# Liupeter01/Software-Rasterizer

Hardware: AMD Instinct MI355X
Metric: frames_per_sec (higher is better)
Workload: dtype f32

## Files before the change

software-rasterizer_amd/csrc/srz_api.hip:

```cpp
#include <dlfcn.h>

#include <algorithm>
#include <cmath>
#include <cstdio>
#include <cstdlib>
#include <cstring>
#include <new>
#include <string>
#include <vector>

#include "srz_device.h"

using namespace srz;

namespace {
std::string g_create_error;

struct EventPair {
  hipEvent_t t0, t1, t2, t3;
  bool detailed;
};

struct BatchDesc {
  int32_t shader, tex_id;
// ... 450 lines not shown
  }
  return SRZ_OK;
}

void end_clear_plan(srz_frameset *fs, const ClearPlan &p, hipStream_t s) {
  if (p.count) ++fs->clear_tune.renders;
  if (p.stamp) launch_clear_tune(fs->clear_tune.d_ctl, fs->clear_tune.h_wgs, s);
  if (p.rebase) launch_clear_rebase(fs->clear_tune.d_ctl, s);
}

struct RenderPlan {
  Pass pass;
  hipStream_t s;
  bool side, turns, vertex_setup;
  ClearPlan clear;
  EventPair *ep;
};

int enqueue_sub_batch(srz_ctx *ctx, srz_frameset *fs, const RenderPlan &r, RenderArgs &a, int f0, int n, int part) {
  const bool stats = r.pass.kind == Pass::COUNTING;
  const hipStream_t s = r.s;
  const size_t tpf = (size_t)fs->n_local_bands * fs->tiles_x;
  RenderArgs v = a;
  if (n != fs->n_frames) {
    const int fa = r.pass.f_begin + f0;
    v.frames += fa, v.n_frames = (uint32_t)n;
    v.vis += (size_t)fa * tpf * ((size_t)TILE * TILE);
    v.tile_info += (size_t)fa * tpf;
    v.out += (size_t)fa * a.frame_stride;
    v.work_cap = (uint32_t)((size_t)(n < 8 ? n : (n + 7) / 8) * tpf);
  }
  const uint32_t tiles = (uint32_t)((size_t)n * tpf);
  if (r.vertex_setup) launch_chunks(v, n, fs->max_tris, s);
  else launch_setup(v, n, fs->max_tris, stats, s);
  launch_bin(v, n, fs->max_tris, s);
  if (!fs->pool_sized && !stats) {
    HIP_TRY(ctx, copy_demand(fs, part, s));
    HIP_TRY(ctx, hipStreamSynchronize(s));
    const uint32_t need = max_pool_demand(fs, part, part + 1);
    if (need > fs->pool_sub_cap) {
      if (int rc = grow_pool(ctx, fs, need, 8u)) return rc;
      a.pool = v.pool = fs->d_pool, a.pool_sub_cap = v.pool_sub_cap = fs->pool_sub_cap;
      HIP_TRY(ctx, hipMemsetAsync(fs->d_pool_heads, 0, sizeof(uint32_t) * CNT_STRIDE * fs->pool_n_sub, s));
      launch_bin(v, n, fs->max_tris, s);
    }
  }
  if (r.pass.kind == Pass::SIZE_ONLY) return SRZ_OK;
  if (r.ep) HIP_TRY(ctx, hipEventRecord(r.ep->t1, s));
  const unsigned ev = r.side ? ctx->ev_next++ % srz_ctx::EV_RING : 0u;
  if (r.side) {
    HIP_TRY(ctx, hipEventRecord(ctx->ev_fork[ev], s));
    HIP_TRY(ctx, hipStreamWaitEvent(ctx->stream2, ctx->ev_fork[ev], 0));
    launch_clear(v, tiles, ctx->stream2, r.clear.wgs);
    HIP_TRY(ctx, copy_demand(fs, part, ctx->stream2));
    HIP_TRY(ctx, hipEventRecord(ctx->ev_join[ev], ctx->stream2));
  }
  launch_raster(v, n, stats, s);
  if (r.turns) {
    HIP_TRY(ctx, hipEventRecord(ctx->ev_raster[ctx->raster_next++ % srz_ctx::EV_RING], s));
    ctx->raster_last_stream = s, ctx->raster_valid = true;
  }
  if (r.ep) HIP_TRY(ctx, hipEventRecord(r.ep->t2, s));
  if (r.pass.kind == Pass::VISIBILITY) launch_visibility(v, tiles, s);
  else launch_shade(v, tiles, stats, fs->fast_kinds, fs->any_generic, fs->approx_shade, s);
  if (r.side) HIP_TRY(ctx, hipStreamWaitEvent(s, ctx->ev_join[ev], 0));
  else if (!raster_four_waves(v))
    HIP_TRY(ctx, copy_demand(fs, part, s));
  return SRZ_OK;
}

int check_renderable(srz_ctx *ctx, const srz_frameset *fs) {
  if (fs->shard_rank != ctx->shard_rank || fs->shard_world != ctx->shard_world)
    return fail(ctx, SRZ_E_INVALID, "frameset was created under a different shard (call srz_set_shard before srz_frameset_create)");
  if (fs->update_failed) return fail(ctx, SRZ_E_NOMEM, "the last update of this set failed (out of memory): update it again or destroy it");
  return SRZ_OK;
}

int render_impl(srz_ctx *ctx, srz_frameset *fs, float *d_out, uint32_t flags_or, hipStream_t s, Pass pass) {
  const bool stats = pass.kind == Pass::COUNTING, size_only = pass.kind == Pass::SIZE_ONLY;
  if (int rc = check_renderable(ctx, fs)) return rc;
  if (pass.kind == Pass::COLOUR || stats)
    if (int rc = resolve_shading(ctx, fs, s)) return rc;
  const uint32_t need = max_pool_demand(fs, 0, srz_frameset::DEMAND_PARTS);
  if (need > fs->pool_sub_cap)
    if (int rc = grow_pool(ctx, fs, need, 4u)) return rc;
  RenderArgs a = make_args(ctx, fs, d_out, flags_or, pass);
  if (!size_only) fs->last_flags = flags_or, fs->rendered = true;
  EventPair ep{};
  const bool timed = ctx->timing != 0 && !stats && !size_only && ctx->ev_used.size() < 65536, detailed = timed && ctx->timing >= 2;
  if (timed)
    if (int rc = begin_timing(ctx, ep, detailed, s)) return rc;
  if (stats) HIP_TRY(ctx, hipMemsetAsync(ctx->d_stats, 0, ST_COUNT * sizeof(unsigned long long), s));
  if (fs->max_tris == 0) {
    HIP_TRY(ctx, hipMemsetAsync(fs->d_work_count, 0, sizeof(uint32_t) * CNT_STRIDE * N_WORK_LISTS, s));
    HIP_TRY(ctx, hipMemsetAsync(fs->d_pool_heads, 0, sizeof(uint32_t) * CNT_STRIDE * fs->pool_n_sub, s));
    HIP_TRY(ctx, hipMemsetAsync(fs->d_slow_count, 0, 2 * sizeof(uint32_t), s));
  }
  const bool turns = !stats && !size_only && fs->max_tiles >= 8192;
  if (turns && !ctx->ev_raster[0])
    if (int rc = create_side(ctx, "render: raster events", nullptr, false, ctx->ev_raster)) return rc;
  if (turns && ctx->raster_valid && ctx->raster_last_stream != s) {
    HIP_TRY(ctx, hipStreamWaitEvent(s, ctx->ev_raster[(ctx->raster_next + srz_ctx::EV_RING - 1) % srz_ctx::EV_RING], 0));
    a.other_streams = 1u;
  }
  const bool vertex_setup = fs->d_draws != nullptr && !stats;
  if (fs->d_draws) launch_vertex(fs->d_draws, fs->n_draws, fs->max_faces, fs->d_tris, fs->d_tri_pos, fs->d_frames, vertex_setup ? fs->d_bbox : nullptr, s);
  const bool any_fused = any_frame_has(fs, flags_or, SRZ_FUSED_CLEAR), side = any_fused && fs->max_tiles >= 8192 && !size_only;
  if (side && !ctx->stream2)
    if (int rc = create_side(ctx, "render: clear stream", &ctx->stream2, true, ctx->ev_fork, ctx->ev_join)) return rc;
  if (!side && any_fused) a.clear_in_raster = 1u;
  RenderPlan r{pass, s, side, turns, vertex_setup, ClearPlan{}, detailed ? &ep : nullptr};
  if (side)
    if (int rc = plan_clear(ctx, fs, pass, detailed, s, r.clear)) return rc;
  a.clear_wgs_dev = r.clear.dev_wgs;
  const int n_all = pass.f_count < 0 ? fs->n_frames : pass.f_count;
  const int chunk = sub_batch_frames(ctx, fs, n_all, stats || detailed);
  for (int f0 = 0, part = 0; f0 < n_all; f0 += chunk, ++part)
    if (int rc = enqueue_sub_batch(ctx, fs, r, a, f0, std::min(chunk, n_all - f0), part)) return rc;
  if (!stats) fs->pool_sized = true;
  end_clear_plan(fs, r.clear, s);
  if (timed) {
    HIP_TRY(ctx, hipEventRecord(ep.t3, s));
    ctx->ev_used.push_back(ep);
  }
  HIP_TRY(ctx, hipGetLastError());
  return SRZ_OK;
}

int render_entry(const char *name, srz_ctx *ctx, srz_frameset *fs, void *d_out, size_t out_bytes, uint32_t flags, void *stream, Pass pass) {
  if (!ctx) return SRZ_E_INVALID;
  const std::string fn(name);
  if (!fs || !d_out) return fail(ctx, SRZ_E_INVALID, fn + ": null frameset / output");
  if (out_bytes < srz_frameset_out_bytes(ctx, fs)) return fail(ctx, SRZ_E_INVALID, fn + ": output buffer too small");
  if (((uintptr_t)d_out & 15u) != 0) return fail(ctx, SRZ_E_INVALID, fn + ": output must be 16-byte aligned");
  HIP_TRY(ctx, hipSetDevice(ctx->device));
  return render_impl(ctx, fs, (float *)d_out, flags & FRAME_FLAGS, pick_stream(ctx, stream), pass);
}

int read_stats(srz_ctx *ctx, hipStream_t s, srz_stats *st) {
  unsigned long long h[ST_COUNT];
  HIP_TRY(ctx, hipMemcpyAsync(h, ctx->d_stats, sizeof h, hipMemcpyDeviceToHost, s));
  HIP_TRY(ctx, hipStreamSynchronize(s));
  st->n_tris = h[ST_TRIS], st->n_culled = h[ST_CULLED], st->pixel_tests = h[ST_PIXEL_TESTS];
  st->fragments = h[ST_FRAGMENTS], st->shaded = h[ST_SHADED], st->visible = h[ST_VISIBLE];
  st->visible_textured = h[ST_VISIBLE_TEX];
  std::memcpy(ctx->dbg, h, sizeof h);
  return SRZ_OK;
// ... 241 lines not shown
      o += sb.n_tris;
    }
    if (fr.n_lights) std::memcpy(&fs->h_lights[d.light_off], fr.lights, sizeof(srz_light) * fr.n_lights);
  }
  classify_frames(fs);
  if (draws) {
    fs->h_draws = *draws, fs->n_draws = (uint32_t)draws->size();
    for (const DrawDesc &dd : *draws) fs->max_faces = std::max(fs->max_faces, dd.n_faces);
  }
  auto up16 = [](size_t v) { return (v + 15) & ~(size_t)15; };
  fs->dyn_lights_off = up16(sizeof(FrameDesc) * (size_t)n_frames);
  fs->dyn_draws_off = up16(fs->dyn_lights_off + sizeof(srz_light) * (size_t)light_off);
  fs->dyn_bytes = fs->dyn_draws_off + sizeof(DrawDesc) * fs->h_draws.size();
  auto dev_alloc = [&](void **p, size_t bytes) { return hipMalloc(p, std::max<size_t>(bytes, 256)); };
  hipError_t e = hipSuccess;
#define FS_TRY(expr)                                                                                                   \
  if (e == hipSuccess) e = (expr)
  FS_TRY(dev_alloc((void **)&fs->d_dyn, fs->dyn_bytes));
  if (e == hipSuccess) {
    fs->d_frames = reinterpret_cast<FrameDesc *>(fs->d_dyn);
    fs->d_lights = reinterpret_cast<srz_light *>(fs->d_dyn + fs->dyn_lights_off);
    if (draws) fs->d_draws = reinterpret_cast<DrawDesc *>(fs->d_dyn + fs->dyn_draws_off);
  }
  FS_TRY(dev_alloc((void **)&fs->d_tris, sizeof(srz_tri) * tri_off));
  if (!fs->tris_aos) FS_TRY(dev_alloc((void **)&fs->d_tri_pos, sizeof(float) * TRI_POS_F * tri_off + 16));
  FS_TRY(dev_alloc((void **)&fs->d_bbox, sizeof(BBox) * tri_off));
  FS_TRY(dev_alloc((void **)&fs->d_chunk_rows, sizeof(uint32_t) * (tri_off / 64 + (size_t)n_frames + 1)));
  FS_TRY(dev_alloc((void **)&fs->d_band_desc, sizeof(uint32_t) * group_off * fs->n_local_bands));
  FS_TRY(dev_alloc((void **)&fs->d_band_ent, sizeof(uint2) * group_off * ENT_PER_GROUP));
  FS_TRY(dev_alloc((void **)&fs->d_tri_batch, sizeof(uint16_t) * tri_off));
  fs->max_tiles = (uint32_t)n_frames * fs->n_local_bands * fs->tiles_x;
  {
    const uint64_t n_wgs = (uint64_t)((n_frames + 7) / 8 * 8) * fs->n_local_bands;
    uint32_t n_sub = 1;
    while (n_sub < 64u && (uint64_t)n_sub * 256u <= n_wgs) n_sub *= 2u;
    fs->pool_n_sub = n_sub;
    const uint64_t cap = std::min<uint64_t>((4ull * tri_off + 4096u) / n_sub + 64u, 0xfffffff0ull / n_sub);
    fs->pool_sub_cap = (uint32_t)cap;
    FS_TRY(dev_alloc((void **)&fs->d_pool, sizeof(uint32_t) * cap * n_sub));
    FS_TRY(dev_alloc((void **)&fs->d_pool_heads, sizeof(uint32_t) * CNT_STRIDE * 64));
    FS_TRY(hipHostMalloc((void **)&fs->h_pool_heads, sizeof(uint32_t) * CNT_STRIDE * 64 * srz_frameset::DEMAND_PARTS, hipHostMallocMapped | hipHostMallocCoherent));
    if (e == hipSuccess) std::memset(fs->h_pool_heads, 0, sizeof(uint32_t) * CNT_STRIDE * 64 * srz_frameset::DEMAND_PARTS);
    FS_TRY(dev_alloc((void **)&fs->clear_tune.d_ctl, sizeof(ClearCtl)));
    if (e == hipSuccess) FS_TRY(hipMemset(fs->clear_tune.d_ctl, 0, sizeof(ClearCtl)));
    FS_TRY(hipHostMalloc((void **)&fs->clear_tune.h_wgs, 64, hipHostMallocMapped | hipHostMallocCoherent));
    if (e == hipSuccess) *fs->clear_tune.h_wgs = 0u;
    FS_TRY(dev_alloc((void **)&fs->d_tile_info, sizeof(uint2) * fs->max_tiles));
    FS_TRY(dev_alloc((void **)&fs->d_slow_list, sizeof(uint32_t) * fs->max_tiles));
    FS_TRY(dev_alloc((void **)&fs->d_slow_count, 2 * sizeof(uint32_t)));
    FS_TRY(dev_alloc((void **)&fs->d_redo_list, sizeof(uint4) * fs->max_tiles));
  }
  FS_TRY(dev_alloc((void **)&fs->d_vis, sizeof(uint32_t) * (size_t)fs->max_tiles * ((size_t)TILE * TILE)));
  FS_TRY(ensure_worklists(fs));
  FS_TRY(dev_alloc((void **)&fs->d_work_count, sizeof(uint32_t) * CNT_STRIDE * N_WORK_LISTS));
  FS_TRY(dev_alloc((void **)&fs->d_sdesc, sizeof(ShadeDescG) * fs->h_batches.size()));
  std::vector<uint8_t> h_dyn(fs->dyn_bytes);
  stage_dyn(fs, h_dyn.data());
  FS_TRY(hipMemcpy(fs->d_dyn, h_dyn.data(), fs->dyn_bytes, hipMemcpyHostToDevice));
  if (tri_off) {
    if (copy_tris) FS_TRY(hipMemcpy(fs->d_tris, h_tris.data(), sizeof(srz_tri) * tri_off, hipMemcpyHostToDevice));
    if (!h_pos.empty()) FS_TRY(hipMemcpy(fs->d_tri_pos, h_pos.data(), sizeof(float) * h_pos.size(), hipMemcpyHostToDevice));
    FS_TRY(hipMemcpy(fs->d_tri_batch, h_tb.data(), sizeof(uint16_t) * tri_off, hipMemcpyHostToDevice));
  }
#undef FS_TRY
  if (e != hipSuccess) {
    free_frameset_buffers(fs);
    delete fs;
    return fail(ctx, e == hipErrorOutOfMemory ? SRZ_E_NOMEM : SRZ_E_NODEVICE,
                std::string("srz_frameset_create: ") + hipGetErrorString(e));
  }
  *out = fs;
  return SRZ_OK;
}

static int size_pool_at_create(srz_ctx *ctx, srz_frameset **out) {
  srz_frameset *fs = *out;
  if (fs->pool_sized) return SRZ_OK;
  int rc = render_impl(ctx, fs, nullptr, 0, ctx->stream, Pass::size_only());
  if (rc == SRZ_OK && hipStreamSynchronize(ctx->stream) != hipSuccess) rc = fail(ctx, SRZ_E_NODEVICE, "srz_frameset_create: the binning pass failed");
  if (rc != SRZ_OK) {
    srz_frameset_destroy(ctx, fs);
    *out = nullptr;
  }
  return rc;
}

int srz_frameset_create(srz_ctx *ctx, const srz_frame *frames, int n_frames, srz_frameset **out) {
  int rc = build_frameset(ctx, frames, n_frames, out, true);
  return rc == SRZ_OK ? size_pool_at_create(ctx, out) : rc;
}

int srz_mesh_upload(srz_ctx *ctx, int mesh_id, const srz_vertex *verts, uint32_t n_verts, const uint32_t *faces, uint32_t n_faces) {
  if (!ctx) return SRZ_E_INVALID;
  if (mesh_id < 0 || mesh_id >= MAX_MESH || !verts || !faces || n_verts == 0) return fail(ctx, SRZ_E_INVALID, "srz_mesh_upload: bad arguments");
  for (uint32_t i = 0; i < 3u * n_faces; ++i)
    if (faces[i] >= n_verts) return fail(ctx, SRZ_E_INVALID, "srz_mesh_upload: face index out of range");
  HIP_TRY(ctx, hipSetDevice(ctx->device));
  srz_ctx::MeshSlot m;
  HIP_TRY(ctx, hipMalloc(&m.d_verts, sizeof(srz_vertex) * n_verts));
  hipError_t e = hipMalloc(&m.d_faces, sizeof(uint32_t) * 3 * (n_faces ? n_faces : 1));
  if (e == hipSuccess) e = hipMemcpy(m.d_verts, verts, sizeof(srz_vertex) * n_verts, hipMemcpyHostToDevice);
  if (e == hipSuccess && n_faces) e = hipMemcpy(m.d_faces, faces, sizeof(uint32_t) * 3 * n_faces, hipMemcpyHostToDevice);
  if (e != hipSuccess) {
    (void)hipFree(m.d_verts), (void)hipFree(m.d_faces);
    return fail(ctx, SRZ_E_NOMEM, std::string("srz_mesh_upload: ") + hipGetErrorString(e));
  }
  m.n_verts = n_verts, m.n_faces = n_faces;
// ... 914 lines not shown
```

software-rasterizer_amd/csrc/srz_device.h:

```cpp
#pragma once
#include <hip/hip_runtime.h>
#include <stdint.h>

#include "../../include/srz.h"

namespace srz {

constexpr int TILE = 32;
constexpr int BAND = 32;
constexpr int KEY_STRIDE = TILE + 1;
constexpr int LDS_STRIDE = 32;
#ifndef SRZ_BAND_ROT
#define SRZ_BAND_ROT 5
#endif
__host__ __device__ inline int band_rot(int world) { return (SRZ_BAND_ROT % world) ? SRZ_BAND_ROT : (SRZ_BAND_ROT ? 1 : 0); }
__host__ __device__ inline int band_of(int lb, int rank, int world) {
  if (world == 1) return lb;
  int j = (rank - band_rot(world) * lb) % world;
  return lb * world + (j < 0 ? j + world : j);
}
__host__ __device__ inline int rank_of_band(int b, int world) { return (b + band_rot(world) * (b / world)) % world; }
constexpr uint32_t NO_TRI = 0xffffffffu;
constexpr uint32_t CNT_STRIDE = 32;
constexpr uint32_t FD_FAST_SHADE = 0x100u, FD_NL_SHIFT = 9;
// ... 56 lines not shown
  uint32_t n_local_bands;
  uint32_t chunk_off;
  uint32_t group_off;
};

enum { ST_TRIS = 0, ST_CULLED, ST_PIXEL_TESTS, ST_FRAGMENTS, ST_SHADED, ST_VISIBLE, ST_VISIBLE_TEX,
       ST_DBG_CYC_A, ST_DBG_CYC_B, ST_DBG_CYC_C, ST_DBG_MAX_WAVE, ST_DBG_IEEE_TILES, ST_DBG_BLOCKS, ST_COUNT };

struct RenderArgs {
  const FrameDesc *frames;
  const srz_tri *tris;
  const float *tri_pos;
  uint32_t pos_stride;
  const BBox *bbox;
  uint32_t *chunk_rows;
  uint32_t *band_desc;
  uint2 *band_ent;
  const uint16_t *tri_batch;
  const srz_light *lights;
  const ShadeDescG *sdesc;
  uint32_t *pool;
  uint32_t *pool_heads;
  uint32_t *pool_demand;
  uint32_t pool_sub_cap, pool_sub_mask;
  uint2 *tile_info;
  uint32_t *slow_list;
  uint32_t *slow_count;
  uint32_t other_streams;
  uint32_t clear_in_raster;
  uint32_t force_ordered;
  uint32_t any_ordered;
  uint32_t force_generic;
  uint32_t any_generic;
  uint4 *redo_list;
  uint32_t *redo_count;
  uint32_t *vis;
  uint4 *worklist;
  uint64_t kind_slots;
  uint32_t *work_count;
  uint32_t work_cap;
  uint32_t tiles_x, n_local_bands, n_frames;
  float *out;
  uint64_t frame_stride;
  uint32_t local_rows;
  int32_t shard_rank, shard_world;
  uint32_t flags_or;
  unsigned long long *stats;
  const uint32_t *clear_wgs_dev;
};

constexpr int CLEAR_CANDS = 3, CLEAR_TUNE_BLOCK = 3, CLEAR_TUNE_RENDERS = 2 * CLEAR_CANDS * CLEAR_TUNE_BLOCK;
constexpr uint32_t CLEAR_CAND[CLEAR_CANDS] = {96, 128, 256};
constexpr uint32_t CLEAR_GRID_MAX = 256, CLEAR_GRID_DEFAULT = 96;
struct ClearCtl {
  uint32_t wgs;
  uint32_t cur, pos, phase, done, alive;
  uint32_t n[CLEAR_CANDS];
  unsigned long long last;
  float t[CLEAR_CANDS][4];
  float score[CLEAR_CANDS];
};
void launch_clear_tune(ClearCtl *ctl, uint32_t *h_wgs, hipStream_t s);
void launch_clear_rebase(ClearCtl *ctl, hipStream_t s);

void launch_vertex(const DrawDesc *draws, uint32_t n_draws, uint32_t max_faces, srz_tri *tris, float *tri_pos, const FrameDesc *frames,
                   BBox *bbox_out, hipStream_t s);
void launch_chunks(const RenderArgs &a, int n_frames, uint32_t max_tris, hipStream_t s);
void launch_setup(const RenderArgs &a, int n_frames, uint32_t max_tris, bool stats, hipStream_t s);
void launch_bin(const RenderArgs &a, int n_frames, uint32_t max_tris, hipStream_t s);
void launch_raster(const RenderArgs &a, int n_frames, bool stats, hipStream_t s);
bool raster_four_waves(const RenderArgs &a);
void launch_clear(const RenderArgs &a, uint32_t max_tiles, hipStream_t s, uint32_t wgs);
void launch_shade(const RenderArgs &a, uint32_t max_tiles, bool stats, uint32_t kinds, bool any_generic, bool approx, hipStream_t s);
void launch_visibility(const RenderArgs &a, uint32_t max_tiles, hipStream_t s);
struct ShadeVisArgs {
  const FrameDesc *frames;
  const srz_tri *tris;
  const uint16_t *tri_batch;
  const srz_light *lights;
  const ShadeDescG *sdesc;
  const float *vis;
  float *out;
  uint64_t frame_stride;
  uint32_t local_rows, tiles_x, n_local_bands, n_frames;
  int32_t shard_rank, shard_world;
  uint32_t flags_or, in_place;
  uint32_t any_generic;
  uint32_t *redo_list;
  uint32_t *redo_count;
};
void launch_shade_vis(const ShadeVisArgs &a, uint32_t kinds, bool any_generic, bool approx, hipStream_t s);
void launch_resolve8(const float *planes, uint8_t *out, uint32_t n_frames, uint32_t rows, uint32_t W, uint64_t frame_stride,
                     hipStream_t s);
void launch_deinterleave(const void *gathered, void *full, uint32_t world, uint32_t n_fp, uint32_t bands_per_rank, uint32_t row_bytes,
                         hipStream_t s);
constexpr uint32_t SPARSE_HEADER = 16;
constexpr uint32_t SPARSE_NONE = 0xffffffffu;
constexpr uint32_t SPARSE_UNPACK_WGS = 2048;
struct SparseArgs {
  const void *shard;
  uint8_t *msg;
  const uint2 *tile_info;
  const FrameDesc *frames;
  uint32_t *row_cnt;
  uint32_t flags_or;
  uint32_t n_frames, n_local_bands, bands_per_rank, tiles_x;
// ... 14 lines not shown
```

software-rasterizer_amd/csrc/srz_kernels.hip:

```cpp
#include "srz_device.h"

#include <algorithm>
#include <cstdio>
#include <cstdlib>
#include <type_traits>

#pragma clang fp contract(off)

namespace srz {

#define SRZ_CAS __attribute__((address_space(4)))
template <typename T> __device__ __forceinline__ const SRZ_CAS T *as_const(const T *p) { return (const SRZ_CAS T *)(p); }
typedef float f32x4 __attribute__((ext_vector_type(4)));
typedef unsigned int u32x2 __attribute__((ext_vector_type(2)));
typedef unsigned int u32x4 __attribute__((ext_vector_type(4)));

__device__ __forceinline__ float sse_max(float a, float b) { return a > b ? a : b; }
__device__ __forceinline__ float sse_min(float a, float b) { return a < b ? a : b; }
__device__ __forceinline__ float std_max(float a, float b) { return (a < b) ? b : a; }
__device__ __forceinline__ float std_clamp(float v, float lo, float hi) { return (v < lo) ? lo : (hi < v) ? hi : v; }
__device__ __forceinline__ float fmsubf(float a, float b, float c) { return __builtin_fmaf(a, b, -c); }
__device__ __forceinline__ float fmaf_(float a, float b, float c) { return __builtin_fmaf(a, b, c); }

__device__ __forceinline__ uint32_t f2u_(float f) { return __builtin_bit_cast(uint32_t, f); }
// ... 432 lines not shown
      run += (uint32_t)__builtin_amdgcn_readlane((int)incl, 63);
    }
    if (lane == 0 && run > ENT_PER_GROUP) s_misc[0] = 1u;
  }
  __syncthreads();
  const bool raw = s_misc[0] != 0u;
  uint32_t tpk[GROUP_K];
#pragma unroll
  for (int k = 0; k < (int)GROUP_K; ++k) {
    const uint32_t t = t0 + (uint32_t)k * 256u + (uint32_t)tid;
    tpk[k] = t;
    if (packed && keep[k]) tpk[k] = t | ((uint32_t)as_const(a.tri_batch)[tri_off + t] << PACK_IDX_BITS);
  }
  uint32_t *desc = a.band_desc + (size_t)group * nlb;
  for (uint32_t i = (uint32_t)tid; i < nlb; i += 256u) desc[i] = raw ? DESC_RAW : ((s_off[i] << 16) | s_cnt[i]);
  if (!raw) {
    uint2 *ent = a.band_ent + (size_t)group * ENT_PER_GROUP;
#pragma unroll
    for (int k = 0; k < (int)GROUP_K; ++k) {
      const uint32_t xr = (uint32_t)((int)bb[k].sx >> 5) | ((uint32_t)((int)bb[k].ex >> 5) << 16);
      float m = 0.0f;
      const bool tight = P != nullptr && nb[k] > 0 &&
                         tight_margin(P[k][0], P[k][1], P[k][3], P[k][4], P[k][6], P[k][7],
                                      (P[k][3] - P[k][0]) * (P[k][7] - P[k][1]) - (P[k][4] - P[k][1]) * (P[k][6] - P[k][0]), bb[k].sx,
                                      bb[k].sy, bb[k].ex, bb[k].ey, m);
      for (int j = 0; j < nb[k]; ++j) {
        uint32_t xr_j = xr;
        if (tight) {
          const int b = band_of(lb0[k] + j, rank, world);
          int X0 = bb[k].sx, X1 = bb[k].ex;
          float mn, mx;
          slab_extent(P[k][0], P[k][1], P[k][3], P[k][4], P[k][6], P[k][7], (float)max(b * BAND, (int)bb[k].sy) - m,
                      (float)min(b * BAND + BAND - 1, (int)bb[k].ey) + m, mn, mx);
          clip_range(X0, X1, mn, mx, m);
          xr_j = X0 <= X1 ? ((uint32_t)(X0 >> 5) | ((uint32_t)(X1 >> 5) << 16)) : 1u;
        }
        ent[atomicAdd(&s_fill[lb0[k] + j], 1u)] = make_uint2(tpk[k], xr_j);
      }
    }
  }
  __syncthreads();
}

__device__ __forceinline__ void chunk_rows_store(const RenderArgs &a, const uint32_t chunk_off, const uint32_t t, const uint32_t n_tris,
                                                 const bool keep, const BBox &bb) {
  int lo = keep ? (int)bb.sy : 0x7fff, hi = keep ? (int)bb.ey : -1;
  for (int o = 32; o > 0; o >>= 1) lo = min(lo, __shfl_xor(lo, o)), hi = max(hi, __shfl_xor(hi, o));
  if ((threadIdx.x & 63) == 0 && (t & ~63u) < n_tris) a.chunk_rows[chunk_off + t / 64u] = ((uint32_t)lo & 0xffffu) | ((uint32_t)hi << 16);
}

__device__ __forceinline__ void reset_render_counters(const RenderArgs &a) {
  if (threadIdx.x < N_WORK_LISTS) a.work_count[threadIdx.x * CNT_STRIDE] = 0u, a.work_count[threadIdx.x * CNT_STRIDE + 1] = 0u;
  if (threadIdx.x <= a.pool_sub_mask) a.pool_heads[threadIdx.x * CNT_STRIDE] = 0u;
  if (threadIdx.x == 0) *a.slow_count = 0u, *a.redo_count = 0u;
}

template <bool STATS>
__global__ __launch_bounds__(256) void k_setup(RenderArgs a, BBox *bbox_out) {
  __shared__ uint32_t s_cnt[MAX_LOCAL_BANDS], s_off[MAX_LOCAL_BANDS], s_fill[MAX_LOCAL_BANDS], s_misc[2];
  if (blockIdx.x == 0 && blockIdx.y == 0) reset_render_counters(a);
  const SRZ_CAS FrameDesc *fd = as_const(a.frames) + blockIdx.y;
  const int W = fd->width, H = fd->height;
  const uint32_t n_tris = fd->n_tris, tri_off = fd->tri_off;
  const float ex = fd->eye[0], ey = fd->eye[1], ez = fd->eye[2];
  unsigned long long n_culled = 0, tests = 0;
  const uint32_t n_groups = (n_tris + GROUP_TRIS - 1u) / GROUP_TRIS;
  for (uint32_t g = blockIdx.x; g < n_groups; g += gridDim.x) {
    const uint32_t t0 = g * GROUP_TRIS;
    float P[GROUP_K][9];
#pragma unroll
    for (int k = 0; k < (int)GROUP_K; ++k) {
      const uint32_t t = t0 + (uint32_t)k * 256u + threadIdx.x;
      load_pos9(as_const(a.tri_pos) + (size_t)(tri_off + (t < n_tris ? t : 0u)) * a.pos_stride, P[k]);
    }
    BBox bb[GROUP_K];
    bool keep[GROUP_K];
#pragma unroll
    for (int k = 0; k < (int)GROUP_K; ++k) {
      const uint32_t t = t0 + (uint32_t)k * 256u + threadIdx.x;
      const bool live = t < n_tris;
      keep[k] = setup_triangle(P[k], W, H, ex, ey, ez, live, bb[k]);
      if (STATS) {
        if (keep[k])
          tests += (unsigned long long)(bb[k].ex - bb[k].sx + 1) * (unsigned long long)(bb[k].ey - bb[k].sy + 1);
        else if (live)
          n_culled++;
      }
      if (live) bbox_out[tri_off + t] = bb[k];
      chunk_rows_store(a, fd->chunk_off, t, n_tris, keep[k], bb[k]);
    }
    bucket_group(a, fd->n_local_bands, fd->group_off + g, t0, (fd->flags & FD_PACKED) != 0u, tri_off, bb, keep, P, s_cnt, s_off, s_fill, s_misc);
  }
  if (STATS) {
    if (n_culled) atomicAdd(&a.stats[ST_CULLED], n_culled);
    if (tests) atomicAdd(&a.stats[ST_PIXEL_TESTS], tests);
    if (blockIdx.x == 0 && threadIdx.x == 0) atomicAdd(&a.stats[ST_TRIS], (unsigned long long)n_tris);
  }
}

__global__ __launch_bounds__(256) void k_chunks(RenderArgs a) {
  __shared__ uint32_t s_cnt[MAX_LOCAL_BANDS], s_off[MAX_LOCAL_BANDS], s_fill[MAX_LOCAL_BANDS], s_misc[2];
  if (blockIdx.x == 0 && blockIdx.y == 0) reset_render_counters(a);
  const SRZ_CAS FrameDesc *fd = as_const(a.frames) + blockIdx.y;
  const uint32_t n_tris = fd->n_tris, tri_off = fd->tri_off;
  const SRZ_CAS u32x2 *bbox = as_const(reinterpret_cast<const u32x2 *>(a.bbox + tri_off));
  const uint32_t n_groups = (n_tris + GROUP_TRIS - 1u) / GROUP_TRIS;
  for (uint32_t g = blockIdx.x; g < n_groups; g += gridDim.x) {
// ... 1187 lines not shown
              const bool pass = inside & !(z > zold);
              if (pass) {
                zl[li] = z;
                il[li] = idx | S_CLASS_BIT;
              }
              if (STATS) n_frag += inside ? 1 : 0, n_shaded += pass ? 1 : 0;
            }
          }
        }
      }
    }
    __builtin_amdgcn_wave_barrier();
    bool any_owner = false;
    for (int it = 0; it < 4; ++it) {
      const uint4 q = *reinterpret_cast<const uint4 *>(&il[(it * 8 + (lane >> 3)) * LDS_STRIDE + (lane & 7) * 4]);
      any_owner |= (q.x & q.y & q.z & q.w) != NO_TRI;
    }
    const bool tile_has_owner = __ballot(any_owner) != 0ull;
    const bool vec_ok = (W & 3) == 0;
    if (tile_has_owner || fused) {
      const float4 zero4 = make_float4(0.f, 0.f, 0.f, 0.f);
      for (int it = 0; it < 4; ++it) {
        const int ly = it * 8 + (lane >> 3), lx4 = (lane & 7) * 4;
        const int y = rc.ty0 + ly, x4 = rc.tx0 + lx4;
        if (y > rc.ty1 || x4 > rc.tx1) continue;
        const float4 z4 = *reinterpret_cast<const float4 *>(&zl[ly * LDS_STRIDE + lx4]);
        float *gz = rc.out0 + (size_t)ly * W + x4;
        const bool full = vec_ok && x4 + 3 <= rc.tx1;
        if (tile_has_owner)
          quad_store(gz, rc.plane, {z4}, full, x4, rc.tx1);
        else
          quad_store(gz, rc.plane, {z4, zero4, zero4, zero4}, full, x4, rc.tx1);
      }
    }
    if (tile_has_owner) {
      uint32_t *slot = a.vis + (size_t)entry * PIX_SLOT;
      for (int it = 0; it < 4; ++it) {
        const int ly = it * 8 + (lane >> 3), lx4 = (lane & 7) * 4;
        ids_store4(slot, (uint32_t)(ly * TILE + lx4), *reinterpret_cast<const uint4 *>(&il[ly * LDS_STRIDE + lx4]), false, false);
      }
      if (lane == 0) work_append(a, fd->flags, entry, work_entry(frame, lb, tx, false, false, 0u, 0u));
    }
    __builtin_amdgcn_wave_barrier();
  }
  if (STATS) {
    for (int o = 32; o > 0; o >>= 1) n_frag += __shfl_down(n_frag, o), n_shaded += __shfl_down(n_shaded, o);
    if (lane == 0) {
      if (n_frag) atomicAdd(&a.stats[ST_FRAGMENTS], n_frag);
      if (n_shaded) atomicAdd(&a.stats[ST_SHADED], n_shaded);
    }
  }
}

__global__ __launch_bounds__(256) void k_clear(RenderArgs a) {
  const uint32_t n_items = a.n_frames * a.n_local_bands * 4u;
  const float inf = __builtin_inff();
  uint32_t n_wgs = gridDim.x;
  if (a.clear_wgs_dev) {
    const uint32_t w = *as_const(a.clear_wgs_dev);
    n_wgs = min(w ? w : CLEAR_CAND[0], gridDim.x);
    if (blockIdx.x >= n_wgs) return;
  }
  for (uint32_t it = blockIdx.x; it < n_items; it += n_wgs) {
    const uint32_t br = it >> 2, pl = it & 3u;
    const uint32_t f = br / a.n_local_bands, lb = br % a.n_local_bands;
    const SRZ_CAS FrameDesc *fd = as_const(a.frames) + f;
    if (!((fd->flags | a.flags_or) & SRZ_FUSED_CLEAR)) continue;
    const int W = fd->width, H = fd->height;
    const int band = band_of((int)lb, a.shard_rank, a.shard_world);
    const int rows = min(BAND, H - band * BAND);
    const size_t plane = (size_t)a.local_rows * (size_t)W;
    float *base = a.out + (size_t)f * a.frame_stride + (size_t)lb * BAND * (size_t)W + pl * plane;
    const float v = pl == 0u ? inf : 0.f;
    const float4 v4 = make_float4(v, v, v, v);
    const SRZ_CAS u32x2 *cnt = as_const(reinterpret_cast<const u32x2 *>(a.tile_info)) + (size_t)br * a.tiles_x;
    for (int x4 = (int)threadIdx.x * 4; x4 < W; x4 += (int)blockDim.x * 4) {
      if (cnt[(uint32_t)x4 / TILE].x != 0u) continue;
      if (((W & 3) == 0)) {
        for (int ly = 0; ly < rows; ++ly) store_nt(base + (size_t)ly * W + x4, v4);
      } else {
        for (int ly = 0; ly < rows; ++ly)
          for (int k = 0; k < 4 && x4 + k < W; ++k) base[(size_t)ly * W + x4 + k] = v;
      }
    }
  }
}


#ifndef SRZ_FAST_MINW
#define SRZ_FAST_MINW 6
#endif
#ifndef SRZ_STAGE_TRIS
#define SRZ_STAGE_TRIS 96
#endif
constexpr uint32_t STAGE_TRIS = SRZ_STAGE_TRIS, STAGE_SD = 16;
static_assert(SRZ_STAGE_TRIS * 6 * 16 >= 2 * 32 * 32 * 4, "SRZ_STAGE_TRIS: s_tri must hold a tile's 1024 {pixel, index} pairs (>= 86 triangles)");
#ifndef SRZ_GENPOW_MINW
#define SRZ_GENPOW_MINW 5
#endif
#ifndef SRZ_SHADE_MINW
#define SRZ_SHADE_MINW 4
#endif
template <bool STATS, int FASTNL, bool BUMPY = false, bool APPROX = false>
__global__ __launch_bounds__(256, (FASTNL > 0 && FASTNL <= 2 && !BUMPY) ? SRZ_FAST_MINW : (FASTNL < 0 && FASTNL >= -2) ? SRZ_GENPOW_MINW
                                  : ((FASTNL == 3 || FASTNL == -3) && !BUMPY) ? 5 : SRZ_SHADE_MINW)
void k_shade(RenderArgs a) {
  constexpr bool FAST = FASTNL != 0, GENPOW = FASTNL < 0;
  static_assert(FAST || !BUMPY, "BUMPY is a property of the FAST builds");
  static_assert(!APPROX || (FASTNL > 0 && !BUMPY && !STATS), "the tolerance mode has FAST builds for 1..4 lights only");
  static_assert(!(GENPOW && BUMPY), "frames with BUMP / DISPLACEMENT batches and a non-integer exponent take the generic build");
  __shared__ __attribute__((aligned(16))) float s_c[3][TILE * TILE];
  __shared__ __attribute__((aligned(16))) uint32_t s_ent[PIX_SLOT];
  __shared__ uint32_t s_wcnt[4];
  __shared__ __attribute__((aligned(16))) f32x4 s_tri[STAGE_TRIS * 6];
  __shared__ uint16_t s_bat[STAGE_TRIS];
  __shared__ __attribute__((aligned(16))) ShadeDescG s_sd[STAGE_SD];
  __shared__ uint32_t s_flag;

  const int tid = threadIdx.x, lane = tid & 63;
  const int wave = __builtin_amdgcn_readfirstlane(tid >> 6);
  unsigned long long n_vis = 0, n_vis_tex = 0;
#ifdef SRZ_PHASE_PROBE
  unsigned long long ph[6] = {0, 0, 0, 0, 0, 0}, ph_t = 0;
  const unsigned long long ph_c0 = __builtin_amdgcn_s_memtime(), ph_r0 = __builtin_amdgcn_s_memrealtime();
#define SRZ_STAMP(K) { const unsigned long long t_ = __builtin_amdgcn_s_memtime(); ph[K] += t_ - ph_t, ph_t = t_; }
#else
#define SRZ_STAMP(K)
#endif

  auto shade_tile = [&](const u32x4 x, auto mode_c) {
    constexpr int MODE = decltype(mode_c)::value;
    int tid = (int)threadIdx.x;
    asm volatile("" : "+v"(tid));
    const int lane = tid & 63;
#ifdef SRZ_PHASE_PROBE
    ph_t = __builtin_amdgcn_s_memtime(), ph[5] += 1;
#endif
    const SRZ_CAS RenderArgs *ap = (const SRZ_CAS RenderArgs *)__builtin_amdgcn_kernarg_segment_ptr();
// ... 1060 lines not shown
      worse = 0.5f * (c->t[c->cur][0] + c->t[c->cur][1]) > 1.05f * best;
    }
    const int tried = (int)c->cur + 1;
    if (tried < CLEAR_CANDS && !worse) next = tried;
    else {
      float m[CLEAR_CANDS];
      int ib = 0;
      for (int i = 0; i < tried; ++i) {
        m[i] = 0.5f * (c->t[i][0] + c->t[i][1]);
        if (m[i] < m[ib]) ib = i;
      }
      for (int i = tried; i < CLEAR_CANDS; ++i) m[i] = 0.f;
      uint32_t alive = 0;
      for (int i = 0; i < tried; ++i)
        if (i <= ib || m[i] <= 1.05f * m[ib]) alive |= 1u << i;
      c->alive = alive, c->phase = 1u;
      for (int i = 0; i < CLEAR_CANDS; ++i) c->score[i] = (alive >> i & 1u) ? m[i] : 0.f;
      if (__popc(alive) > 1) next = 31 - __clz((int)alive);
    }
  } else {
    const uint32_t lower = c->alive & ((1u << c->cur) - 1u);
    if (lower) next = 31 - __clz((int)lower);
    else
      for (int i = 0; i < CLEAR_CANDS; ++i)
        if (c->alive >> i & 1u) {
          float *t = c->t[i];
          for (int x = 1; x < 4; ++x)
            for (int y = x; y > 0 && t[y] < t[y - 1]; --y) { const float u = t[y]; t[y] = t[y - 1], t[y - 1] = u; }
          c->score[i] = 0.5f * (t[1] + t[2]);
        }
  }
  if (next >= 0) {
    c->cur = (uint32_t)next, c->wgs = CLEAR_CAND[next];
    return;
  }
  int arg = -1;
  for (int i = 0; i < CLEAR_CANDS; ++i)
    if ((c->alive >> i & 1u) && (arg < 0 || c->score[i] < c->score[arg])) arg = i;
  c->wgs = CLEAR_CAND[arg < 0 ? 0 : arg], c->done = 1u;
  __hip_atomic_store(h_wgs, c->wgs, __ATOMIC_RELEASE, __HIP_MEMORY_SCOPE_SYSTEM);
}

void launch_clear_tune(ClearCtl *ctl, uint32_t *h_wgs, hipStream_t s) { hipLaunchKernelGGL(k_clear_tune, dim3(1), dim3(1), 0, s, ctl, h_wgs); }

__global__ void k_clear_rebase(ClearCtl *c) {
  if (!c->done) c->last = __builtin_amdgcn_s_memrealtime();
}
void launch_clear_rebase(ClearCtl *ctl, hipStream_t s) { hipLaunchKernelGGL(k_clear_rebase, dim3(1), dim3(1), 0, s, ctl); }

void launch_clear(const RenderArgs &a, uint32_t max_tiles, hipStream_t s, uint32_t wgs) {
  if (max_tiles == 0) return;
  const uint32_t n_items = a.n_frames * a.n_local_bands * 4u;
  const uint32_t cap = wgs ? wgs : 96u;
  hipLaunchKernelGGL(k_clear, dim3(n_items < cap ? n_items : cap), dim3(256), 0, s, a);
}

static dim3 shade_grid(const RenderArgs &a, uint32_t max_tiles) {
  return dim3((std::min(max_tiles, a.other_streams ? 2048u : 16384u) + 7u) & ~7u);
}

template <int FASTNL, bool BUMPY, class L> static void launch_kind(uint32_t kinds, bool approx, L &launch) {
  if (!((kinds >> build_kind<FASTNL, BUMPY>()) & 1u)) return;
  if constexpr (FASTNL > 0 && !BUMPY)
    if (approx) return launch(std::integral_constant<int, FASTNL>{}, std::false_type{}, std::true_type{});
  launch(std::integral_constant<int, FASTNL>{}, std::bool_constant<BUMPY>{}, std::false_type{});
}
template <class L> static void launch_fast_kinds(uint32_t kinds, bool approx, L &&launch) {
  launch_kind<1, false>(kinds, approx, launch), launch_kind<2, false>(kinds, approx, launch);
  launch_kind<3, false>(kinds, approx, launch), launch_kind<4, false>(kinds, approx, launch);
  launch_kind<1, true>(kinds, approx, launch), launch_kind<2, true>(kinds, approx, launch);
  launch_kind<3, true>(kinds, approx, launch), launch_kind<4, true>(kinds, approx, launch);
  launch_kind<-1, false>(kinds, approx, launch), launch_kind<-2, false>(kinds, approx, launch);
  launch_kind<-3, false>(kinds, approx, launch), launch_kind<-4, false>(kinds, approx, launch);
}

void launch_shade(const RenderArgs &a, uint32_t max_tiles, bool stats, uint32_t kinds, bool any_generic, bool approx, hipStream_t s) {
  if (max_tiles == 0) return;
  const dim3 grid = shade_grid(a, max_tiles);
  if (stats) {
    hipLaunchKernelGGL((k_shade<true, 0>), grid, dim3(256), 0, s, a);
    return;
  }
  launch_fast_kinds(kinds, approx, [&](auto nl, auto bumpy, auto ap) {
    hipLaunchKernelGGL((k_shade<false, decltype(nl)::value, decltype(bumpy)::value, decltype(ap)::value>), grid, dim3(256), 0, s, a);
  });
  dim3 ggrid(any_generic ? grid.x : (grid.x < 128u ? grid.x : 128u));
  hipLaunchKernelGGL((k_shade<false, 0>), ggrid, dim3(256), 0, s, a);
}

void launch_visibility(const RenderArgs &a, uint32_t max_tiles, hipStream_t s) {
  if (max_tiles == 0) return;
  hipLaunchKernelGGL(k_visibility, shade_grid(a, max_tiles), dim3(256), 0, s, a);
}

void launch_shade_vis(const ShadeVisArgs &a, uint32_t kinds, bool any_generic, bool approx, hipStream_t s) {
  const uint32_t items = a.n_frames * a.n_local_bands * a.tiles_x;
  if (items == 0) return;
  const dim3 grid((std::min(items, 16384u) + 7u) & ~7u), blk(256);
  launch_fast_kinds(kinds, approx, [&](auto nl, auto bumpy, auto ap) {
    hipLaunchKernelGGL((k_shade_vis<decltype(nl)::value, decltype(bumpy)::value, decltype(ap)::value>), grid, blk, 0, s, a);
  });
  if (any_generic || (kinds && !approx)) hipLaunchKernelGGL((k_shade_vis<0>), any_generic ? grid : dim3(std::min(grid.x, 128u)), blk, 0, s, a);
}

bool raster_four_waves(const RenderArgs &a) { return a.n_frames * a.n_local_bands * a.tiles_x <= 4096u; }

void launch_raster(const RenderArgs &a, int n_frames, bool stats, hipStream_t s) {
// ... 21 lines not shown
```

Before: 330,100.

## Hand out clear work items dynamically via atomic ticket and move demand copy

The fused-clear kernel no longer uses a static round-robin over items. Each block now carries an extra dealer wave that takes the next item from a global atomic ticket counter and passes it to the workers through double-buffered shared memory, which should balance uneven per-band clear costs. The ticket word is stored after the work counters and reset together with them. The demand-count copy leaves the side clear stream and now runs on the main stream after shading. This adds a __syncthreads per item and an idle wave per block, and it may lengthen the main stream. An optional probe for timing per-block clear work sits behind a macro.

```diff
diff --git a/software-rasterizer_amd/csrc/srz_api.hip b/software-rasterizer_amd/csrc/srz_api.hip
--- a/software-rasterizer_amd/csrc/srz_api.hip
+++ b/software-rasterizer_amd/csrc/srz_api.hip
@@ -526,7 +526,6 @@
     HIP_TRY(ctx, hipEventRecord(ctx->ev_fork[ev], s));
     HIP_TRY(ctx, hipStreamWaitEvent(ctx->stream2, ctx->ev_fork[ev], 0));
     launch_clear(v, tiles, ctx->stream2, r.clear.wgs);
-    HIP_TRY(ctx, copy_demand(fs, part, ctx->stream2));
     HIP_TRY(ctx, hipEventRecord(ctx->ev_join[ev], ctx->stream2));
   }
   launch_raster(v, n, stats, s);
@@ -537,9 +536,9 @@
   if (r.ep) HIP_TRY(ctx, hipEventRecord(r.ep->t2, s));
   if (r.pass.kind == Pass::VISIBILITY) launch_visibility(v, tiles, s);
   else launch_shade(v, tiles, stats, fs->fast_kinds, fs->any_generic, fs->approx_shade, s);
+  if (r.side || !raster_four_waves(v))
+    HIP_TRY(ctx, copy_demand(fs, part, s));
   if (r.side) HIP_TRY(ctx, hipStreamWaitEvent(s, ctx->ev_join[ev], 0));
-  else if (!raster_four_waves(v))
-    HIP_TRY(ctx, copy_demand(fs, part, s));
   return SRZ_OK;
 }
 
@@ -566,7 +565,7 @@
     if (int rc = begin_timing(ctx, ep, detailed, s)) return rc;
   if (stats) HIP_TRY(ctx, hipMemsetAsync(ctx->d_stats, 0, ST_COUNT * sizeof(unsigned long long), s));
   if (fs->max_tris == 0) {
-    HIP_TRY(ctx, hipMemsetAsync(fs->d_work_count, 0, sizeof(uint32_t) * CNT_STRIDE * N_WORK_LISTS, s));
+    HIP_TRY(ctx, hipMemsetAsync(fs->d_work_count, 0, sizeof(uint32_t) * WORK_COUNT_WORDS, s));
     HIP_TRY(ctx, hipMemsetAsync(fs->d_pool_heads, 0, sizeof(uint32_t) * CNT_STRIDE * fs->pool_n_sub, s));
     HIP_TRY(ctx, hipMemsetAsync(fs->d_slow_count, 0, 2 * sizeof(uint32_t), s));
   }
@@ -914,7 +913,7 @@
   }
   FS_TRY(dev_alloc((void **)&fs->d_vis, sizeof(uint32_t) * (size_t)fs->max_tiles * ((size_t)TILE * TILE)));
   FS_TRY(ensure_worklists(fs));
-  FS_TRY(dev_alloc((void **)&fs->d_work_count, sizeof(uint32_t) * CNT_STRIDE * N_WORK_LISTS));
+  FS_TRY(dev_alloc((void **)&fs->d_work_count, sizeof(uint32_t) * WORK_COUNT_WORDS));
   FS_TRY(dev_alloc((void **)&fs->d_sdesc, sizeof(ShadeDescG) * fs->h_batches.size()));
   std::vector<uint8_t> h_dyn(fs->dyn_bytes);
   stage_dyn(fs, h_dyn.data());
diff --git a/software-rasterizer_amd/csrc/srz_device.h b/software-rasterizer_amd/csrc/srz_device.h
--- a/software-rasterizer_amd/csrc/srz_device.h
+++ b/software-rasterizer_amd/csrc/srz_device.h
@@ -132,6 +132,7 @@
 constexpr int CLEAR_CANDS = 3, CLEAR_TUNE_BLOCK = 3, CLEAR_TUNE_RENDERS = 2 * CLEAR_CANDS * CLEAR_TUNE_BLOCK;
 constexpr uint32_t CLEAR_CAND[CLEAR_CANDS] = {96, 128, 256};
 constexpr uint32_t CLEAR_GRID_MAX = 256, CLEAR_GRID_DEFAULT = 96;
+constexpr uint32_t CLEAR_THREADS = 256, CLEAR_TICKET_WORD = N_WORK_LISTS * CNT_STRIDE, WORK_COUNT_WORDS = CLEAR_TICKET_WORD + CNT_STRIDE;
 struct ClearCtl {
   uint32_t wgs;
   uint32_t cur, pos, phase, done, alive;
diff --git a/software-rasterizer_amd/csrc/srz_kernels.hip b/software-rasterizer_amd/csrc/srz_kernels.hip
--- a/software-rasterizer_amd/csrc/srz_kernels.hip
+++ b/software-rasterizer_amd/csrc/srz_kernels.hip
@@ -508,7 +508,7 @@
 __device__ __forceinline__ void reset_render_counters(const RenderArgs &a) {
   if (threadIdx.x < N_WORK_LISTS) a.work_count[threadIdx.x * CNT_STRIDE] = 0u, a.work_count[threadIdx.x * CNT_STRIDE + 1] = 0u;
   if (threadIdx.x <= a.pool_sub_mask) a.pool_heads[threadIdx.x * CNT_STRIDE] = 0u;
-  if (threadIdx.x == 0) *a.slow_count = 0u, *a.redo_count = 0u;
+  if (threadIdx.x == 0) *a.slow_count = 0u, *a.redo_count = 0u, a.work_count[CLEAR_TICKET_WORD] = 0u;
 }
 
 template <bool STATS>
@@ -1802,7 +1802,17 @@
   }
 }
 
-__global__ __launch_bounds__(256) void k_clear(RenderArgs a) {
+#ifdef SRZ_CLEAR_PROBE
+__device__ unsigned long long g_clear_probe[CLEAR_GRID_MAX * 4u];
+extern "C" __attribute__((visibility("default"))) int srz_debug_clear_probe(unsigned long long *out, int n_words) {
+  if (hipDeviceSynchronize() != hipSuccess) return -1;
+  const size_t n = std::min((size_t)std::max(n_words, 0), (size_t)CLEAR_GRID_MAX * 4u);
+  return hipMemcpyFromSymbol(out, HIP_SYMBOL(g_clear_probe), n * sizeof(unsigned long long)) == hipSuccess ? (int)n : -1;
+}
+#endif
+
+__global__ __launch_bounds__(CLEAR_THREADS + 64) void k_clear(RenderArgs a) {
+  __shared__ uint32_t s_next[2];
   const uint32_t n_items = a.n_frames * a.n_local_bands * 4u;
   const float inf = __builtin_inff();
   uint32_t n_wgs = gridDim.x;
@@ -1811,7 +1821,26 @@
     n_wgs = min(w ? w : CLEAR_CAND[0], gridDim.x);
     if (blockIdx.x >= n_wgs) return;
   }
-  for (uint32_t it = blockIdx.x; it < n_items; it += n_wgs) {
+  const bool dealer = threadIdx.x >= CLEAR_THREADS;
+#ifdef SRZ_CLEAR_PROBE
+  const unsigned long long probe_t0 = __builtin_amdgcn_s_memrealtime();
+  uint32_t probe_items = 0;
+#endif
+  uint32_t par = 0;
+  auto next_item = [&]() {
+    __syncthreads();
+    const uint32_t t = s_next[par];
+    par ^= 1u;
+    return t;
+  };
+  for (uint32_t it = blockIdx.x; it < n_items; it = next_item()) {
+#ifdef SRZ_CLEAR_PROBE
+    ++probe_items;
+#endif
+    if (dealer) {
+      if (threadIdx.x == CLEAR_THREADS) s_next[par] = n_wgs + atomicAdd(a.work_count + CLEAR_TICKET_WORD, 1u);
+      continue;
+    }
     const uint32_t br = it >> 2, pl = it & 3u;
     const uint32_t f = br / a.n_local_bands, lb = br % a.n_local_bands;
     const SRZ_CAS FrameDesc *fd = as_const(a.frames) + f;
@@ -1824,7 +1853,7 @@
     const float v = pl == 0u ? inf : 0.f;
     const float4 v4 = make_float4(v, v, v, v);
     const SRZ_CAS u32x2 *cnt = as_const(reinterpret_cast<const u32x2 *>(a.tile_info)) + (size_t)br * a.tiles_x;
-    for (int x4 = (int)threadIdx.x * 4; x4 < W; x4 += (int)blockDim.x * 4) {
+    for (int x4 = (int)threadIdx.x * 4; x4 < W; x4 += (int)CLEAR_THREADS * 4) {
       if (cnt[(uint32_t)x4 / TILE].x != 0u) continue;
       if (((W & 3) == 0)) {
         for (int ly = 0; ly < rows; ++ly) store_nt(base + (size_t)ly * W + x4, v4);
@@ -1834,6 +1863,12 @@
       }
     }
   }
+#ifdef SRZ_CLEAR_PROBE
+  if (threadIdx.x == 0) {
+    unsigned long long *p = g_clear_probe + (size_t)blockIdx.x * 4u;
+    p[0] = probe_t0, p[1] = __builtin_amdgcn_s_memrealtime(), p[2] = probe_items, p[3] = n_wgs;
+  }
+#endif
 }
 
 
@@ -3000,7 +3035,7 @@
   if (max_tiles == 0) return;
   const uint32_t n_items = a.n_frames * a.n_local_bands * 4u;
   const uint32_t cap = wgs ? wgs : 96u;
-  hipLaunchKernelGGL(k_clear, dim3(n_items < cap ? n_items : cap), dim3(256), 0, s, a);
+  hipLaunchKernelGGL(k_clear, dim3(n_items < cap ? n_items : cap), dim3(CLEAR_THREADS + 64), 0, s, a);
 }
 
 static dim3 shade_grid(const RenderArgs &a, uint32_t max_tiles) {
```

Result: slower. 326,100 (-1.2%).
